# kallenordling/cesm_emulator

Measured on NVIDIA B200. Metric: train samples/s (baseline cfg), higher is better.
Workload: dtype fp16

## Files before the change

cesm_emulator_b200/_lib.py:

```python
from __future__ import annotations

import ctypes
from ctypes import POINTER, Structure, c_char_p, c_float, c_int32, c_int64, c_void_p
from pathlib import Path

_PKG = Path(__file__).resolve().parent
LIB_PATH = _PKG / "libcesm_b200.so"

CESM_MAX_TAPS = 16


class IgemmArgs(Structure):

    _fields_ = [
        ("a0", c_void_p), ("a1", c_void_p),
        ("c0", c_int32), ("c1", c_int32),
        ("n", c_int32), ("h", c_int32), ("w", c_int32),
        ("stride", c_int32),
        ("num_taps", c_int32),
        ("tap_dh", c_int32 * CESM_MAX_TAPS), ("tap_dw", c_int32 * CESM_MAX_TAPS),
        ("wt", c_void_p), ("cout", c_int32),
        ("oh", c_int32), ("ow", c_int32),
        ("out", c_void_p), ("ldo", c_int32),
        ("out_h", c_int32), ("out_w", c_int32),
# ... 62 lines not shown
    lib.cesm_adamw_partials.restype = ctypes.c_int
    lib.cesm_tattn_long_max_frames.restype = ctypes.c_int
    lib.cesm_set_prezeroed_scratch.restype = None
    lib.cesm_set_prezeroed_scratch.argtypes = [ctypes.c_int]
    _declare(lib)
    _lib = lib
    return lib


_P, _I, _L, _F, _U = c_void_p, ctypes.c_int, ctypes.c_longlong, c_float, ctypes.c_uint
_SIGNATURES: dict[str, list] = {
    "cesm_igemm": [POINTER(IgemmArgs), _P],
    "cesm_wgrad": [POINTER(WgradArgs), _P],
    "cesm_pack_weight": [_P, _P, _I, _I, _I, _L, _L, POINTER(c_int32), _P],
    "cesm_pack_weights_batched": [_P, _I, _P],
    "cesm_unpack_wgrads_batched": [_P, _I, _P],
    "cesm_unpack_wgrad": [_P, _P, _I, _I, _I, _L, _L, POINTER(c_int32), _I, _P],
    "cesm_adamw_step": [_P, _P, _P, _P, _L, _P, _P, _F, _F, _F, _F, _P],
    "cesm_adamw_ema_step": [_P, _P, _P, _P, _P, _L, _P, _P, _F, _F, _F, _F, ctypes.c_double, _L, _P],
    "cesm_colsum": [_P, _P, _L, _I, _I, _P],
    "cesm_gn_stats": [_P, _P, _I, _L, _I, _I, _P],
    "cesm_gn_apply_fwd": [_P, _P, _P, _P, _P, _P, _P, _I, _L, _I, _I, _F, _P],
    "cesm_gn_bwd": [_P, _P, _P, _P, _P, _P, _P, _P, _P, _P, _P, _P, _I, _L, _I, _I, _F, _I, _P],
    "cesm_ln_fwd": [_P, _P, _P, _L, _I, _F, _P],
    "cesm_ln_bwd": [_P, _P, _P, _P, _P, _P, _L, _I, _F, _I, _P],
    "cesm_tattn_fwd": [_P, _P, _P, _P, _P, _P, _I, _I, _I, _I, _I, _F, _P],
    "cesm_tattn_bwd": [_P, _P, _P, _P, _P, _P, _P, _P, _P, _I, _I, _I, _I, _I, _F, _P],
    "cesm_tattn_proj_fwd": [_P, _P, _P, _P, _P, _P, _I, _I, _I, _I, _I, _I, _F, _P],
    "cesm_tattn_long_fwd": [_P, _P, _P, _P, _P, _P, _I, _I, _I, _I, _I, _F, _P],
    "cesm_tattn_long_bwd": [_P, _P, _P, _P, _P, _P, _P, _P, _P, _I, _I, _I, _I, _I, _F, _P],
# ... 105 lines not shown
```

cesm_emulator_b200/csrc/api_common.h:

```cpp
#pragma once
#include <cuda.h>
#include <cuda_runtime.h>
#include <stdarg.h>
#include <stdint.h>

#include "../../include/cesm_b200.h"

namespace cesm {

int set_error(int code, const char* fmt, ...);
#define CESM_CHECK_CUDA(expr)                                                                  \
    do {                                                                                       \
        cudaError_t _e = (expr);                                                               \
        if (_e != cudaSuccess)                                                                 \
            return ::cesm::set_error(CESM_ERR_CUDA, "%s failed: %s (%s:%d)", #expr,            \
                                     cudaGetErrorString(_e), __FILE__, __LINE__);              \
    } while (0)
void note_launch();
#define CESM_CHECK_LAUNCH()            \
    do {                               \
        ::cesm::note_launch();         \
        CESM_CHECK_CUDA(cudaGetLastError()); \
    } while (0)
bool scratch_prezeroed();
#define CESM_ZERO_SCRATCH(ptr, bytes, st)                                               \
    do {                                                                                \
        if (!::cesm::scratch_prezeroed()) CESM_CHECK_CUDA(cudaMemsetAsync((ptr), 0, (bytes), (st))); \
    } while (0)
#define CESM_REQUIRE(cond, ...)                                                 \
    do {                                                                        \
        if (!(cond)) return ::cesm::set_error(CESM_ERR_INVALID, __VA_ARGS__);   \
    } while (0)

template <typename... KArgs, typename... Args>
inline cudaError_t launch_pdl(void (*kern)(KArgs...), dim3 grid, dim3 block, size_t smem, cudaStream_t st, Args... args) {
    cudaLaunchConfig_t cfg = {};
    cfg.gridDim = grid;
    cfg.blockDim = block;
    cfg.dynamicSmemBytes = smem;
    cfg.stream = st;
    cudaLaunchAttribute attr[1];
    attr[0].id = cudaLaunchAttributeProgrammaticStreamSerialization;
    attr[0].val.programmaticStreamSerializationAllowed = 1;
    cfg.attrs = attr;
    cfg.numAttrs = 1;
    return cudaLaunchKernelEx(&cfg, kern, static_cast<KArgs>(args)...);
}

template <typename... KArgs, typename... Args>
inline cudaError_t launch_pdl_cluster(void (*kern)(KArgs...), dim3 grid, dim3 block, size_t smem, cudaStream_t st,
                                      int cluster_x, Args... args) {
    cudaLaunchConfig_t cfg = {};
    cfg.gridDim = grid;
    cfg.blockDim = block;
    cfg.dynamicSmemBytes = smem;
    cfg.stream = st;
    cudaLaunchAttribute attr[2];
    attr[0].id = cudaLaunchAttributeProgrammaticStreamSerialization;
    attr[0].val.programmaticStreamSerializationAllowed = 1;
    int n = 1;
    if (cluster_x > 1) {
        attr[n].id = cudaLaunchAttributeClusterDimension;
        attr[n].val.clusterDim.x = (unsigned)cluster_x;
        attr[n].val.clusterDim.y = 1;
        attr[n].val.clusterDim.z = 1;
        ++n;
    }
    cfg.attrs = attr;
    cfg.numAttrs = n;
    return cudaLaunchKernelEx(&cfg, kern, static_cast<KArgs>(args)...);
}

int get_tensor_map_h16(CUtensorMap* out, const void* base, int rank, const uint64_t* dims,
                        const uint64_t* strides_bytes, const uint32_t* box);
// ... 6 lines not shown
```

cesm_emulator_b200/csrc/api_core.cu:

```cuda
#include <atomic>
#include <mutex>
#include <string>
#include <unordered_map>

#include "api_common.h"
#include "igemm.h"

namespace cesm {

static thread_local std::string g_last_error;
static std::atomic<long long> g_launches{0};
void note_launch() { g_launches.fetch_add(1, std::memory_order_relaxed); }
static std::atomic<int> g_prezeroed{0};
bool scratch_prezeroed() { return g_prezeroed.load(std::memory_order_relaxed) != 0; }

int set_error(int code, const char* fmt, ...) {
    char buf[1024];
    va_list ap;
    va_start(ap, fmt);
    vsnprintf(buf, sizeof(buf), fmt, ap);
    va_end(ap);
    g_last_error = buf;
    return code;
}

typedef CUresult (*EncodeTiledFn)(CUtensorMap*, CUtensorMapDataType, cuuint32_t, void*, const cuuint64_t*,
                                  const cuuint64_t*, const cuuint32_t*, const cuuint32_t*, CUtensorMapInterleave,
                                  CUtensorMapSwizzle, CUtensorMapL2promotion, CUtensorMapFloatOOBfill);

// ... 101 lines not shown
        }
    }
    *bw = b_w;
    *bh = b_h;
    *bn = b_n;
}

}

using namespace cesm;

extern "C" const char* cesm_last_error(void) { return g_last_error.c_str(); }
extern "C" const char* cesm_version(void) { return "cesm_b200 0.1 sm_100a"; }
extern "C" void cesm_set_prezeroed_scratch(int on) { g_prezeroed.store(on ? 1 : 0, std::memory_order_relaxed); }
extern "C" long long cesm_launch_count(void) { return g_launches.load(std::memory_order_relaxed); }

static int sm_count() {
    static int n = 0;
    if (n == 0) {
        int dev = 0, v = 0;
        if (cudaGetDevice(&dev) == cudaSuccess &&
            cudaDeviceGetAttribute(&v, cudaDevAttrMultiProcessorCount, dev) == cudaSuccess && v > 0)
            n = v;
        else
            n = 148;
    }
    return n;
}

static bool is_3x3_unit_taps(const cesm_igemm_args* a) {
// ... 73 lines not shown
                     "bad GroupNorm statistics arguments (groups=%d frames=%d)", a->gn_groups, a->gn_frames);
        p.gn_groups = a->gn_groups;
        p.gn_cpg = a->cout / a->gn_groups;
        p.gn_frames = a->gn_frames;
        CESM_REQUIRE(a->gn_groups <= 32, "fused GroupNorm statistics support at most 32 groups (got %d)", a->gn_groups);
        CESM_REQUIRE(p.gn_cpg % 8 == 0 && (p.gn_cpg >= 64 ? p.gn_cpg % 64 == 0 : 64 % p.gn_cpg == 0),
                     "fused GroupNorm statistics need 8 | cout/groups and cout/groups | 64 or 64 | cout/groups (got %d)",
                     p.gn_cpg);
        if (p.bn > 1 && a->gn_frames % p.bn != 0) {
            p.bn = 1;
            p.m_tiles = p.tiles_w * p.tiles_h * a->n;
        }
        CESM_ZERO_SCRATCH(a->gn_sums, sizeof(float) * 2 * (a->n / a->gn_frames) * a->gn_groups, st);
    }

    const int pw = halo ? p.bw + 2 : p.bw;
    if (halo) {
        const int rows_box = pw * (p.bh + 2), rows_need = 2 * pw + 2 + 128;
        const int rows = rows_box > rows_need ? rows_box : rows_need;
        p.a_stage_bytes = (uint32_t)((rows * 128 + 1023) / 1024 * 1024);
        p.a_box_bytes = (uint32_t)rows_box * 128u;
    } else {
        p.a_stage_bytes = 16384;
        p.a_box_bytes = 128u * p.bw * p.bh * p.bn;
    }
    const long long budget = (long long)kIgemm2MaxSmem - 1024  - 1024  - 2 * 16384 ;
    const long long b_total = (long long)a->cout * p.num_kb * 128 / (pair ? 2 : 1);
    const long long b_blk = (long long)block_n * 128 / (pair ? 2 : 1);
    const int a_min = 2;
    if (b_total + a_min * (long long)p.a_stage_bytes <= budget) {
        p.b_resident = 1;
        p.b_stages = 1;
        long long as = (budget - b_total) / p.a_stage_bytes;
        const int a_cap = halo ? 4 : 8;
        p.a_stages = (int)(as > a_cap ? a_cap : as);
    } else {
        p.b_resident = 0;
        p.a_stages = halo ? 2 : 4;
        long long bs = (budget - (long long)p.a_stages * p.a_stage_bytes) / b_blk;
        if (bs > 16) bs = 16;
        if (bs < 2) {
            p.a_stages = 2;
            bs = (budget - (long long)p.a_stages * p.a_stage_bytes) / b_blk;
        }
        CESM_REQUIRE(bs >= 2, "igemm2: no shared-memory plan for cout=%d K=%d", a->cout, p.num_kb * 64);
        p.b_stages = (int)bs;
// ... 72 lines not shown
                                 (uint64_t)a->out_h * a->out_w * a->ldo * 2};
        if (halo)
            p.epi_warp = (pw == 32);
        else
            p.epi_warp = (p.bw % 32 == 0);
        uint32_t obox[4] = {64u, (uint32_t)p.bw, (uint32_t)(halo ? 1 : p.bh), (uint32_t)(halo ? 1 : p.bn)};
        if (p.epi_warp && !halo) {
            obox[1] = 32u;
            obox[2] = 1u;
            obox[3] = 1u;
        }
        int rc = get_tensor_map_h16(&maps.out, base, 4, dims, str, obox);
        if (rc) return rc;
    }
    p.m_major = p.b_resident && p.n_tiles > 1 ? 1 : 0;
    int grid;
    if (pair) {
        const int units = ((p.m_tiles + 1) / 2) * p.n_tiles, clusters = sm_count() / 2;
        grid = 2 * (units < clusters ? units : clusters);
    } else {
        const int total_tiles = p.m_tiles * p.n_tiles;
        grid = total_tiles < sm_count() ? total_tiles : sm_count();
    }
    note_launch();
    CESM_CHECK_CUDA(igemm2_launch(maps, p, block_n, halo, pair, grid, smem, st));
    return CESM_OK;
}

extern "C" int cesm_igemm(const cesm_igemm_args* a, void* stream) {
    CESM_REQUIRE(a != nullptr, "args is NULL");
    CESM_REQUIRE(a->c0 > 0 && a->c0 % 64 == 0 && a->c1 >= 0 && a->c1 % 64 == 0,
                 "channel counts must be multiples of 64 (c0=%d c1=%d)", a->c0, a->c1);
    CESM_REQUIRE(a->cout > 0 && a->cout % 64 == 0, "cout=%d must be a multiple of 64", a->cout);
    CESM_REQUIRE(a->num_taps >= 1 && a->num_taps <= CESM_MAX_TAPS, "num_taps=%d out of range", a->num_taps);
    CESM_REQUIRE(a->stride == 1 || a->stride == 2, "stride=%d unsupported", a->stride);
    CESM_REQUIRE(a->stride == 1 || (a->c1 == 0 && a->h % 2 == 0 && a->w % 2 == 0),
                 "stride 2 needs a single source with even h, w");
    CESM_REQUIRE(a->n > 0 && a->h > 0 && a->w > 0 && a->oh > 0 && a->ow > 0, "empty geometry");
// ... 209 lines not shown
```

cesm_emulator_b200/csrc/elementwise.cu:

```cuda
#include "api_common.h"
#include "common.cuh"

namespace cesm {

struct TapOffsets {
    int32_t off[CESM_MAX_TAPS];
};

__global__ void pack_weight_kernel(const float* __restrict__ src, h16* __restrict__ dst, int O, int T, int I,
                                   long long so, long long si, TapOffsets taps) {
    pdl_trigger();
    pdl_wait();
    const long long idx = (long long)blockIdx.x * blockDim.x + threadIdx.x;
    if (idx >= (long long)O * T * I) return;
    const int i = idx % I;
    const int t = (idx / I) % T;
    const int o = idx / ((long long)I * T);
    dst[idx] = __float2half_rn(src[o * so + i * si + taps.off[t]]);
}
__global__ void unpack_wgrad_kernel(const float* __restrict__ src, float* __restrict__ dst, int O, int T, int I,
                                    long long so, long long si, TapOffsets taps, int accumulate) {
    pdl_trigger();
    pdl_wait();
    const long long idx = (long long)blockIdx.x * blockDim.x + threadIdx.x;
// ... 847 lines not shown

}

using namespace cesm;

static inline int nblk(long long total, int threads) { return (int)((total + threads - 1) / threads); }

extern "C" int cesm_pack_weight(const float* src, void* dst, int O, int T, int I, long long so, long long si,
                                const int32_t* tap_off, void* stream) {
    CESM_REQUIRE(T >= 1 && T <= CESM_MAX_TAPS, "T=%d out of range", T);
    TapOffsets taps{};
    for (int t = 0; t < T; ++t) taps.off[t] = tap_off[t];
    const long long total = (long long)O * T * I;
    launch_pdl(pack_weight_kernel, nblk(total, 256), 256, 0, as_stream(stream), src, (h16*)dst, O, T, I, so, si, taps);
    CESM_CHECK_LAUNCH();
    return CESM_OK;
}

extern "C" int cesm_unpack_wgrad(const float* src, float* dst, int O, int T, int I, long long so, long long si,
                                 const int32_t* tap_off, int accumulate, void* stream) {
    CESM_REQUIRE(T >= 1 && T <= CESM_MAX_TAPS, "T=%d out of range", T);
    TapOffsets taps{};
    for (int t = 0; t < T; ++t) taps.off[t] = tap_off[t];
    const long long total = (long long)O * T * I;
    launch_pdl(unpack_wgrad_kernel, nblk(total, 256), 256, 0, as_stream(stream), src, dst, O, T, I, so, si, taps, accumulate);
    CESM_CHECK_LAUNCH();
    return CESM_OK;
}

extern "C" int cesm_colsum(const void* x, float* out, long long M, int C, int accumulate, void* stream) {
// ... 22 lines not shown
                                  int W, int ks, int kpad, void* stream) {
    CESM_REQUIRE(ks == 7 && kpad == 256, "input patch kernel is specialised for 7x7, 256 columns (ks=%d kpad=%d)", ks, kpad);
    CESM_REQUIRE((f0 == 1 || f0 == F) && (f1 == 1 || f1 == F), "frame counts must be 1 or F");
    dim3 grid(ceil_div(W, 16), ceil_div(H, 16), B * F);
    launch_pdl(input_patches_kernel<7, 256>, grid, 256, 0, as_stream(stream), in0, in1, f0, f1, (h16*)out, F, H, W);
    CESM_CHECK_LAUNCH();
    return CESM_OK;
}

extern "C" int cesm_input_weight_pack(const float* w, const float* bias, void* out, int cout, int ks, int kpad,
                                      void* stream) {
    CESM_REQUIRE(kpad >= 4 * ks * ks + 2, "kpad=%d too small for 2 planes x hi/lo x %dx%d + 2", kpad, ks, ks);
    launch_pdl(input_weight_pack_kernel, nblk((long long)cout * kpad, 256), 256, 0, as_stream(stream), 
        w, bias, (h16*)out, cout, 2 * ks * ks, kpad);
    CESM_CHECK_LAUNCH();
    return CESM_OK;
}

extern "C" int cesm_input_conv_fwd(const float* in0, const float* in1, int f0, int f1, const float* w,
                                   const float* bias, void* out, int B, int F, int H, int W, int ks, int cout,
                                   void* stream) {
    CESM_REQUIRE(ks == 7 && cout == 64, "input conv kernel is specialised for 7x7, 64 channels (ks=%d cout=%d)", ks, cout);
    CESM_REQUIRE((f0 == 1 || f0 == F) && (f1 == 1 || f1 == F), "frame counts must be 1 or F");
    dim3 grid(ceil_div(W, 16), ceil_div(H, 16), B * F);
    launch_pdl(input_conv_fwd_kernel<7, 64>, grid, 256, 0, as_stream(stream), in0, in1, f0, f1, w, bias, (h16*)out, F, H, W);
    CESM_CHECK_LAUNCH();
    return CESM_OK;
}

extern "C" int cesm_input_conv_wgrad(const float* in0, const float* in1, int f0, int f1, const void* dy, float* dw,
// ... 298 lines not shown
```

cesm_emulator_b200/csrc/igemm.h:

```cpp
#pragma once
#include <cuda.h>
#include <cuda_runtime.h>
#include <stdint.h>

namespace cesm {

struct WgradParams {
    int32_t c0, c1;
    int32_t num_taps;
    int32_t tap_map[16];
    int32_t tap_dh[16];
    int32_t tap_dw[16];
    int32_t n, oh, ow;
    int32_t bw, bh, bn;
    uint32_t box_bytes;
    int32_t cout;
    float* dw;
    long long so, si;
    int32_t tap_off[16];
};

struct Wgrad3Maps {
    CUtensorMap x[2];
    CUtensorMap y;
// ... 19 lines not shown
    CUtensorMap b;
    CUtensorMap out;
};

struct Igemm2Params {
    int32_t c0, c1;
    int32_t num_taps, num_kb;
    int32_t tap_map[16];
    int32_t tap_dh[16];
    int32_t tap_dw[16];
    int32_t n, oh, ow;
    int32_t bw, bh, bn;
    int32_t tiles_w, tiles_h, m_tiles, n_tiles;
    int32_t cout;
    int32_t a_stages, b_stages, b_resident;
    uint32_t a_stage_bytes, a_box_bytes;
    int32_t out_h, out_w, o_sh, o_sw, o_h0, o_w0;
    const float* bias;
    const void* residual;
    int32_t ldr;
    float* gn_sums;
    int32_t gn_groups, gn_cpg, gn_frames;
    int32_t epi_warp;
    int32_t m_major;
    const float* ln_colsum;
    float ln_eps;
};

cudaError_t igemm2_launch(const Igemm2Maps& maps, const Igemm2Params& p, int block_n, bool halo, bool pair, int grid,
                          size_t smem, cudaStream_t stream);
// ... 6 lines not shown
```

cesm_emulator_b200/csrc/igemm2.cu:

```cuda

#include "api_common.h"
#include "common.cuh"
#include "igemm.h"

#include <type_traits>

namespace cesm {

static constexpr int kTileM = 128;
static constexpr int kKBlk = 64;
static constexpr int kStageRowBytes = 128;
static constexpr int kOutStageBytes = kTileM * kStageRowBytes;
static constexpr int kIgemm2Threads = 352;

__device__ __forceinline__ void tma_store_4d(const void* map, uint32_t smem_src, int c0, int c1, int c2, int c3) {
    asm volatile("cp.async.bulk.tensor.4d.global.shared::cta.bulk_group [%0, {%2, %3, %4, %5}], [%1];"
                 :
                 : "l"(reinterpret_cast<uint64_t>(map)), "r"(smem_src), "r"(c0), "r"(c1), "r"(c2), "r"(c3)
                 : "memory");
}
__device__ __forceinline__ void tma_store_commit() { asm volatile("cp.async.bulk.commit_group;" ::: "memory"); }
template <int N>
__device__ __forceinline__ void tma_store_wait_read() {
    asm volatile("cp.async.bulk.wait_group.read %0;" ::"n"(N) : "memory");
}
__device__ __forceinline__ void tma_store_wait_all() { asm volatile("cp.async.bulk.wait_group 0;" ::: "memory"); }
__device__ __forceinline__ void epi_bar_sync(int group) {
    asm volatile("bar.sync %0, 128;" ::"r"(group + 1) : "memory");
// ... 23 lines not shown
igemm2_kernel(const __grid_constant__ Igemm2Maps maps, const Igemm2Params p) {
    static_assert(!PAIR || HALO, "CTA pairs are wired for the 3x3 halo mode only");
    static_assert(!LNF || (BLOCK_N == 64 && !HALO && !GN && !PAIR), "the LayerNorm fold is a 64-column plain GEMM epilogue");
    pdl_trigger();
    extern __shared__ uint8_t smem_raw[];
    const uint32_t smem_base = (smem_u32(smem_raw) + 1023u) & ~1023u;
    uint8_t* smem_gen = smem_raw + (smem_base - smem_u32(smem_raw));

    const uint32_t a_base = smem_base;
    const uint32_t b_base = a_base + p.a_stages * p.a_stage_bytes;
    constexpr int kBRows = PAIR ? BLOCK_N / 2 : BLOCK_N;
    const uint32_t b_blk_bytes = kBRows * kStageRowBytes;
    const uint32_t cta_rank = PAIR ? cluster_ctarank() : 0u;
    const int work_id = PAIR ? (int)(blockIdx.x >> 1) : (int)blockIdx.x;
    const int work_stride = PAIR ? (int)(gridDim.x >> 1) : (int)gridDim.x;
    const uint32_t b_bytes = p.b_resident ? (uint32_t)p.n_tiles * p.num_kb * b_blk_bytes : p.b_stages * b_blk_bytes;
    const uint32_t o_base = b_base + b_bytes;
    const uint32_t bar_base = o_base + 2 * kOutStageBytes;
    auto a_full = [&](int s) { return bar_base + 8u * s; };
    auto a_empty = [&](int s) { return bar_base + 8u * (8 + s); };
    auto b_full = [&](int s) { return bar_base + 8u * (16 + s); };
    auto b_empty = [&](int s) { return bar_base + 8u * (32 + s); };
    auto t_full = [&](int s) { return bar_base + 8u * (48 + s); };
    auto t_empty = [&](int s) { return bar_base + 8u * (50 + s); };
    const uint32_t b_all_bar = bar_base + 8u * 52;
    const uint32_t tmem_ptr_addr = bar_base + 8u * 53;
    const uint32_t gn_base = bar_base + 8u * 56;
    volatile uint32_t* tmem_ptr_gen = reinterpret_cast<volatile uint32_t*>(smem_gen + (tmem_ptr_addr - smem_base));

    const int warp = threadIdx.x >> 5;
    const int lane = threadIdx.x & 31;

    const int cblk0 = p.c0 >> 6;
    const int cblk = (p.c0 + p.c1) >> 6;
    const int a_loads = HALO ? cblk : p.num_kb;
    const int taps_per_a = HALO ? 9 : 1;
    const int pw = HALO ? p.bw + 2 : p.bw;
    const int m_units = PAIR ? (p.m_tiles + 1) >> 1 : p.m_tiles;
    const int total_tiles = m_units * p.n_tiles;
    constexpr uint32_t kTmemCols = (2 * BLOCK_N < 32) ? 32 : 2 * BLOCK_N;

    if (threadIdx.x == 0) {
        tma_prefetch_desc(&maps.a[0]);
        tma_prefetch_desc(&maps.b);
        tma_prefetch_desc(&maps.out);
        for (int s = 0; s < p.a_stages; ++s) {
            mbar_init(a_full(s), 1);
            mbar_init(a_empty(s), 1);
        }
        for (int s = 0; s < p.b_stages; ++s) {
            mbar_init(b_full(s), 1);
            mbar_init(b_empty(s), 1);
        }
        for (int s = 0; s < 2; ++s) {
            mbar_init(t_full(s), 1);
            mbar_init(t_empty(s), (BLOCK_N == 64 ? 4 : 8) * (PAIR ? 2 : 1));
        }
        mbar_init(b_all_bar, 1);
        fence_barrier_init();
    }
    if (threadIdx.x < 128) reinterpret_cast<float*>(smem_gen + (gn_base - smem_base))[threadIdx.x] = 0.f;
    if (warp == 2) {
        if (PAIR) tmem_alloc_pair(tmem_ptr_addr, kTmemCols);
        else tmem_alloc(tmem_ptr_addr, kTmemCols);
    }
    tc_fence_before();
    if (PAIR) cluster_sync_all();
    else __syncthreads();
    tc_fence_after();
    const uint32_t tmem_base = *tmem_ptr_gen;

    auto tile_coords = [&](int tile, int& n_tile, int& n0, int& oh0, int& ow0) {
        int t;
// ... 2 lines not shown
            n_tile = tile - t * p.n_tiles;
        } else {
            n_tile = tile / m_units;
            t = tile - n_tile * m_units;
        }
        if (PAIR) t = 2 * t + (int)cta_rank;
        const int tw = t % p.tiles_w;
        t /= p.tiles_w;
        const int th = t % p.tiles_h;
        const int tn = t / p.tiles_h;
        ow0 = tw * p.bw;
        oh0 = th * p.bh;
        n0 = tn * p.bn;
    };

    if (warp == 0 && lane == 0) {
        pdl_wait();
        int stage = 0;
        uint32_t phase = 0;
        for (int tile = work_id; tile < total_tiles; tile += work_stride) {
            int n_tile, n0, oh0, ow0;
            tile_coords(tile, n_tile, n0, oh0, ow0);
            for (int ai = 0; ai < a_loads; ++ai) {
                mbar_wait(a_empty(stage), phase ^ 1u, 11);
                const uint32_t dst = a_base + stage * p.a_stage_bytes;
                if (PAIR) {
                    if (cta_rank == 0) mbar_arrive_expect_tx(a_full(stage), 2 * p.a_box_bytes);
                    int midx = 0, c = ai << 6;
                    if (ai >= cblk0) {
                        midx = 1;
                        c = (ai - cblk0) << 6;
// ... 27 lines not shown
                    stage = 0;
                    phase ^= 1u;
                }
            }
        }
        if (PAIR) {
            for (int k = 0; k < p.a_stages; ++k) {
                mbar_wait(a_empty(stage), phase ^ 1u, 18);
                if (++stage == p.a_stages) {
                    stage = 0;
                    phase ^= 1u;
                }
            }
        }
    } else if (warp == 1 && lane == 0) {
        pdl_wait();
        const int row_off = (int)cta_rank * kBRows;
        if (p.b_resident) {
            const uint32_t total_bytes = (uint32_t)p.n_tiles * p.num_kb * b_blk_bytes;
            if (cta_rank == 0) mbar_arrive_expect_tx(b_all_bar, (PAIR ? 2u : 1u) * total_bytes);
            for (int nt = 0; nt < p.n_tiles; ++nt)
                for (int kb = 0; kb < p.num_kb; ++kb) {
                    const uint32_t dst = b_base + (nt * p.num_kb + kb) * b_blk_bytes;
                    if (PAIR) tma_load_2d_pair(dst, &maps.b, b_all_bar, kb * kKBlk, nt * BLOCK_N + row_off);
                    else tma_load_2d(dst, &maps.b, b_all_bar, kb * kKBlk, nt * BLOCK_N);
                }
        } else {
            int stage = 0;
            uint32_t phase = 0;
            for (int tile = work_id; tile < total_tiles; tile += work_stride) {
                const int n_tile = p.m_major ? tile % p.n_tiles : tile / m_units;
                for (int ai = 0; ai < a_loads; ++ai)
                    for (int ti = 0; ti < taps_per_a; ++ti) {
                        const int kb = HALO ? ti * cblk + ai : ai;
                        mbar_wait(b_empty(stage), phase ^ 1u, 12);
                        if (PAIR) {
                            if (cta_rank == 0) mbar_arrive_expect_tx(b_full(stage), 2 * b_blk_bytes);
                            tma_load_2d_pair(b_base + stage * b_blk_bytes, &maps.b, b_full(stage), kb * kKBlk,
                                             n_tile * BLOCK_N + row_off);
                            if (++stage == p.b_stages) {
                                stage = 0;
                                phase ^= 1u;
                            }
                            continue;
                        }
                        mbar_arrive_expect_tx(b_full(stage), b_blk_bytes);
                        tma_load_2d(b_base + stage * b_blk_bytes, &maps.b, b_full(stage), kb * kKBlk, n_tile * BLOCK_N);
                        if (++stage == p.b_stages) {
                            stage = 0;
                            phase ^= 1u;
                        }
                    }
            }
            if (PAIR) {
                for (int k = 0; k < p.b_stages; ++k) {
                    mbar_wait(b_empty(stage), phase ^ 1u, 19);
                    if (++stage == p.b_stages) {
                        stage = 0;
                        phase ^= 1u;
                    }
                }
            }
        }
    } else if (warp == 2) {
        if (cta_rank == 0 && elect_one()) {
            constexpr uint32_t idesc = make_idesc_f16(PAIR ? 2 * kTileM : kTileM, BLOCK_N, 0, 0);
            const uint64_t desc_hi = make_smem_desc_sw128(0, 0, 1024);
            uint32_t tap_rows8[9];
#pragma unroll
            for (int ti = 0; ti < 9; ++ti)
                tap_rows8[ti] = HALO ? ((1 + p.tap_dh[ti]) * pw + (1 + p.tap_dw[ti])) * 8 : 0;
            const uint32_t b_blk16 = b_blk_bytes >> 4;
            const uint32_t a_stage16 = p.a_stage_bytes >> 4;
            const uint32_t a_base16 = a_base >> 4, b_base16 = b_base >> 4;
            const uint32_t tap_b16 = cblk * b_blk16;
            const uint32_t tile_b16 = p.num_kb * b_blk16;
            const int n_a_stages = p.a_stages, n_b_stages = p.b_stages, n_tiles = p.n_tiles;
            const bool m_major = p.m_major != 0;
            auto mma4 = [&](uint32_t d_tmem, uint32_t a16, uint32_t b16, uint32_t first_accum) {
#pragma unroll
                for (int k = 0; k < kKBlk / 16; ++k) {
                    const uint64_t da = desc_hi | (uint64_t)(a16 + 2 * k), db = desc_hi | (uint64_t)(b16 + 2 * k);
                    if (PAIR) umma_f16_pair(d_tmem, da, db, idesc, k == 0 ? first_accum : 1u);
                    else umma_f16(d_tmem, da, db, idesc, k == 0 ? first_accum : 1u);
                }
            };
            auto commit = [&](uint32_t bar) {
                if (PAIR) umma_commit_pair(bar);
                else umma_commit(bar);
            };
            auto run = [&](auto resident_tag) {
                constexpr bool RES = decltype(resident_tag)::value;
                int a_stage = 0, b_stage = 0, acc = 0;
                uint32_t a_phase = 0, b_phase = 0, acc_phase = 0;
                if (RES) mbar_wait(b_all_bar, 0, 13);
                for (int tile = work_id; tile < total_tiles; tile += work_stride) {
                    const int n_tile = m_major ? tile % n_tiles : tile / m_units;
                    mbar_wait(t_empty(acc), acc_phase ^ 1u, 14);
                    tc_fence_after();
                    const uint32_t d_tmem = tmem_base + acc * BLOCK_N;
                    uint32_t b_kb16 = b_base16 + n_tile * tile_b16;
                    for (int ai = 0; ai < a_loads; ++ai, b_kb16 += b_blk16) {
                        mbar_wait(a_full(a_stage), a_phase, 15);
                        tc_fence_after();
                        const uint32_t sa16 = a_base16 + a_stage * a_stage16;
                        const uint32_t first = ai != 0;
                        if (RES) {
                            if (HALO) {
                                uint32_t b16 = b_kb16;
#pragma unroll
                                for (int ti = 0; ti < 9; ++ti, b16 += tap_b16)
                                    mma4(d_tmem, sa16 + tap_rows8[ti], b16, ti == 0 ? first : 1u);
                            } else {
                                mma4(d_tmem, sa16, b_kb16, first);
                            }
                        } else {
#pragma unroll
                            for (int ti = 0; ti < (HALO ? 9 : 1); ++ti) {
// ... 2 lines not shown
                                mma4(d_tmem, sa16 + tap_rows8[ti], b_base16 + b_stage * b_blk16, ti == 0 ? first : 1u);
                                commit(b_empty(b_stage));
                                if (++b_stage == n_b_stages) {
                                    b_stage = 0;
                                    b_phase ^= 1u;
                                }
                            }
                        }
                        commit(a_empty(a_stage));
                        if (++a_stage == n_a_stages) {
                            a_stage = 0;
                            a_phase ^= 1u;
                        }
                    }
                    commit(t_full(acc));
                    if (++acc == 2) {
                        acc = 0;
                        acc_phase ^= 1u;
                    }
                }
            };
            if (p.b_resident) run(std::true_type{});
            else run(std::false_type{});
        }
        __syncwarp();
    } else if (warp >= 3) {
        const int q = warp & 3;
        const int group = (warp - 3) >> 2;
        const int r = q * 32 + lane;
        const bool grp_issuer = (lane == 0) && (warp == 3 || warp == 7);
        const bool warp_mode = p.epi_warp != 0;
        const uint32_t obuf = o_base + group * kOutStageBytes;
        const uint32_t my_row = obuf + r * kStageRowBytes;
        const uint32_t sw7 = (r & 7);
        float* gn_acc = reinterpret_cast<float*>(smem_gen + (gn_base - smem_base)) + 64 * group;
        int acc = 0;
        uint32_t acc_phase = 0;
        int cur_b = -1;
        auto gn_flush = [&](int b) {
            epi_bar_sync(group);
            if (q == 3 && b >= 0) {
// ... 45 lines not shown
        auto run_flush = [&]() {
            if (run_key < 0) return;
            const int b = run_key / p.n_tiles, nt = run_key - b * p.n_tiles;
            const int col = nt * BLOCK_N + (BLOCK_N == 64 ? 0 : group * 64);
            const int idx = butterfly16(racc);
            if ((lane & 1) == 0) {
                const int g = (col + 8 * (idx & 7)) / p.gn_cpg;
                atomicAdd(p.gn_sums + ((size_t)b * p.gn_groups + g) * 2 + (idx >> 3), racc[0]);
            }
#pragma unroll
            for (int i = 0; i < 16; ++i) racc[i] = 0.f;
        };
        const int rw = r % pw;
        const int rh = (r / pw) % p.bh;
        const int rn = r / (pw * p.bh);
        const int r0 = q * 32;
        const int st_w = HALO ? 0 : r0 % p.bw, st_h = HALO ? q : (r0 / p.bw) % p.bh, st_n = HALO ? 0 : r0 / (p.bw * p.bh);
        const bool st_ok = HALO ? (q < p.bh) : (st_n < p.bn);
        int tile_it = 0;
        for (int tile = work_id; tile < total_tiles; tile += work_stride, ++tile_it) {
            if (BLOCK_N == 64) {
                if ((tile_it & 1) != group) continue;
                acc = group;
                acc_phase = (tile_it >> 1) & 1;
            }
            int n_tile, n0, oh0, ow0;
            tile_coords(tile, n_tile, n0, oh0, ow0);
            if (PAIR && n0 >= p.n) {
                mbar_wait(t_full(acc), acc_phase, 17);
                tc_fence_after();
// ... 13 lines not shown
            if (GN) {
                const int b = n0 / p.gn_frames;
                if (kRunningStats) {
                    const int key = b * p.n_tiles + n_tile;
                    if (key != run_key) {
                        run_flush();
                        run_key = key;
                    }
                } else if (b != cur_b) {
                    if (cur_b >= 0) gn_flush(cur_b);
                    cur_b = b;
                }
            }
            mbar_wait(t_full(acc), acc_phase, 17);
            tc_fence_after();
            const uint32_t taddr = tmem_base + acc * BLOCK_N + (static_cast<uint32_t>(q * 32) << 16);
            const int last_cc = BLOCK_N == 64 ? 0 : group * 64 + (BLOCK_N > 128 ? 128 : 0);
            bool released = false;
#pragma unroll 1
            for (int cc = (BLOCK_N == 64 ? 0 : group * 64); cc < BLOCK_N; cc += 128) {
                uint32_t v[64];
                tmem_ld_32x64(taddr + cc, v);
                if (warp_mode) {
                    if (lane == 0) tma_store_wait_read<0>();
                    __syncwarp();
                } else {
                    if (grp_issuer) tma_store_wait_read<0>();
                    epi_bar_sync(group);
                }
                const int col = n_tile * BLOCK_N + cc;
// ... 180 lines not shown
```

cesm_emulator_b200/csrc/optim.cu:

```cuda
#include "api_common.h"
#include "common.cuh"

namespace cesm {

static constexpr int kRelayoutThreads = 256;
static constexpr int kTile = 32;
static constexpr int kRelayoutSmem = kTile * (kTile * 9 + 1) * (int)sizeof(float);

__device__ __forceinline__ void cp_async4(uint32_t dst, const void* src) {
    asm volatile("cp.async.ca.shared.global [%0], [%1], 4;" ::"r"(dst), "l"(src) : "memory");
}
__device__ __forceinline__ void cp_async_wait_all() { asm volatile("cp.async.wait_all;" ::: "memory"); }

template <int MODE>
__global__ void __launch_bounds__(kRelayoutThreads)
relayout_tiled_kernel(const cesm_pack_desc* __restrict__ descs) {
    pdl_trigger();
    pdl_wait();
    extern __shared__ float tile[];
    __shared__ int s_off[CESM_MAX_TAPS];
    const cesm_pack_desc& d = descs[blockIdx.y];
    const long long so = d.so, si = d.si;
    const int O = d.O, T = d.T, I = d.I;
    const bool inner_is_i = si < so;
// ... 195 lines not shown

static int relayout_launch(const cesm_pack_desc* descs_device, int n, int mode, cudaStream_t st) {
    constexpr int kSmem = kRelayoutSmem;
    static bool cfg = false;
    if (!cfg) {
        CESM_CHECK_CUDA(cudaFuncSetAttribute(relayout_tiled_kernel<0>, cudaFuncAttributeMaxDynamicSharedMemorySize, kSmem));
        CESM_CHECK_CUDA(cudaFuncSetAttribute(relayout_tiled_kernel<1>, cudaFuncAttributeMaxDynamicSharedMemorySize, kSmem));
        cfg = true;
    }
    dim3 grid(32, n);
    if (mode == 0)
        launch_pdl(relayout_tiled_kernel<0>, grid, kRelayoutThreads, kSmem, st, descs_device);
    else
        launch_pdl(relayout_tiled_kernel<1>, grid, kRelayoutThreads, kSmem, st, descs_device);
    CESM_CHECK_LAUNCH();
    return CESM_OK;
}

extern "C" int cesm_pack_weights_batched(const cesm_pack_desc* descs_device, int n, void* stream) {
    if (n <= 0) return CESM_OK;
    return relayout_launch(descs_device, n, 0, as_stream(stream));
}

extern "C" int cesm_unpack_wgrads_batched(const cesm_pack_desc* descs_device, int n, void* stream) {
    if (n <= 0) return CESM_OK;
    return relayout_launch(descs_device, n, 1, as_stream(stream));
}

extern "C" int cesm_adamw_partials(void) { return 148 * 4; }

// ... 35 lines not shown
```

cesm_emulator_b200/kernels.py:

```python
from __future__ import annotations

import ctypes
import numbers
from typing import Optional, Sequence, Tuple

import torch

from . import _lib
from ._lib import IgemmArgs

H16 = torch.float16


def _stream() -> ctypes.c_void_p:
    return ctypes.c_void_p(torch.cuda.current_stream().cuda_stream)


def _ptr(t: Optional[torch.Tensor]) -> Optional[int]:
    return None if t is None else t.data_ptr()


def _req_cuda(*ts: Optional[torch.Tensor]) -> None:
    for t in ts:
        if t is not None and not t.is_cuda:
# ... 406 lines not shown
              h, w, _stream())


INPUT_KPAD = 256


def input_patches(in0, in1, B: int, F: int, H: int, W: int, ks: int) -> torch.Tensor:
    _req_cuda(in0, in1)
    f0, f1 = in0.numel() // (B * H * W), in1.numel() // (B * H * W)
    out = torch.empty((B * F, H, W, INPUT_KPAD), dtype=H16, device=in0.device)
    _lib.call("cesm_input_patches", _ptr(in0), _ptr(in1), f0, f1, _ptr(out), B, F, H, W, ks, INPUT_KPAD, _stream(),
              _meta=_bytes_meta(out))
    return out


def input_weight_pack(w, bias, out: Optional[torch.Tensor] = None) -> torch.Tensor:
    _req_cuda(w, bias)
    cout, ks = w.shape[0], w.shape[-1]
    if out is None:
        out = torch.empty((cout, INPUT_KPAD), dtype=H16, device=w.device)
    _lib.call("cesm_input_weight_pack", _ptr(w), _ptr(bias), _ptr(out), cout, ks, INPUT_KPAD, _stream())
    return out


def input_conv_fwd(in0, in1, w, bias, B: int, F: int, H: int, W: int, ks: int):
    _req_cuda(in0, in1, w, bias)
    cout = w.shape[0]
    f0, f1 = in0.numel() // (B * H * W), in1.numel() // (B * H * W)
    out = torch.empty((B * F, H, W, cout), dtype=H16, device=in0.device)
    _lib.call("cesm_input_conv_fwd", _ptr(in0), _ptr(in1), f0, f1, _ptr(w), _ptr(bias), _ptr(out), B, F, H, W, ks, cout,
# ... 306 lines not shown
```

cesm_emulator_b200/ops.py:

```python
from __future__ import annotations

import weakref
from typing import Optional, Tuple

import torch

from . import _lib
from . import kernels as K

H16 = torch.float16

_PHASE_TAPS = {0: [(0, 1), (-1, 3)], 1: [(1, 0), (0, 2)]}


_OUTER_GRAD = [True]


class _Fn(torch.autograd.Function):
    @classmethod
    def apply(cls, *args, **kwargs):
        _OUTER_GRAD[0] = torch.is_grad_enabled()
        return super().apply(*args, **kwargs)


# ... 95 lines not shown
    return len(live)


_FOLDS: list = []


def _fold_compute(ent, wqkv, wout, gamma) -> None:
    C, hidden = ent[1].shape[0], ent[4]
    wv = wqkv.detach().reshape(3 * hidden, C)[2 * hidden:].float()
    wo = wout.detach().reshape(C, hidden).float()
    w = wo @ wv
    ent[1].copy_(w)
    if gamma is not None:
        ent[6].copy_(w * gamma.detach().reshape(1, C).float())
        ent[7].copy_(ent[6].float().sum(dim=1))


def _fold_f1(meta, wqkv, wout, hidden: int, C: int, gamma=None):
    key = (_key(wqkv), _key(wout), None if gamma is None else _key(gamma))
    ent = meta.__dict__.get("fold_f1")
    if ent is None or ent[1].device != wqkv.device or (gamma is not None and ent[5] is None):
        dev = wqkv.device
        ent = [None, torch.empty((C, C), dtype=H16, device=dev), weakref.ref(wqkv), weakref.ref(wout), hidden,
               None if gamma is None else weakref.ref(gamma),
               None if gamma is None else torch.empty((C, C), dtype=H16, device=dev),
               None if gamma is None else torch.empty((C,), dtype=torch.float32, device=dev)]
        meta.__dict__["fold_f1"] = ent
        _FOLDS.append(ent)
    if ent[0] != key:
        _fold_compute(ent, wqkv, wout, gamma)
# ... 804 lines not shown
```

include/cesm_b200.h:

```cpp
#ifndef CESM_B200_H
#define CESM_B200_H

#include <stddef.h>
#include <stdint.h>

#ifdef __cplusplus
extern "C" {
#endif

typedef enum cesm_status {
    CESM_OK = 0,
    CESM_ERR_INVALID = -1,
    CESM_ERR_CUDA = -2,
    CESM_ERR_INTERNAL = -3
} cesm_status;

const char* cesm_last_error(void);
const char* cesm_version(void);
long long cesm_launch_count(void);


#define CESM_MAX_TAPS 16

typedef struct cesm_igemm_args {
// ... 42 lines not shown
    int32_t dw_tap_off[CESM_MAX_TAPS];
} cesm_wgrad_args;

int cesm_wgrad(const cesm_wgrad_args* args, void* stream);

int cesm_pack_weight(const float* src, void* dst, int O, int T, int I, long long so, long long si,
                     const int32_t* tap_off, void* stream);
typedef struct cesm_pack_desc {
    const float* src;
    void* dst;
    int32_t O, T, I, pad_;
    long long so, si;
    int32_t tap_off[CESM_MAX_TAPS];
} cesm_pack_desc;
int cesm_pack_weights_batched(const cesm_pack_desc* descs_device, int n, void* stream);
int cesm_unpack_wgrads_batched(const cesm_pack_desc* descs_device, int n, void* stream);
int cesm_qkv_bwd(const void* dy, const void* x, const void* wt, void* dx, float* dw, long long dw_so, long long rows,
                 int cin, int cout, void* stream);

void cesm_set_prezeroed_scratch(int on);

#define CESM_OPT_STATE_FLOATS 16
int cesm_adamw_partials(void);
int cesm_adamw_step(float* p, const float* g, float* m, float* v, long long n, float* partials, float* state,
                    float beta1, float beta2, float eps, float max_norm, void* stream);
int cesm_adamw_ema_step(float* p, const float* g, float* m, float* v, float* ema, long long n, float* partials,
                        float* state, float beta1, float beta2, float eps, float max_norm, double ema_decay,
                        long long ema_start, void* stream);
int cesm_unpack_wgrad(const float* src, float* dst, int O, int T, int I, long long so, long long si,
                      const int32_t* tap_off, int accumulate, void* stream);
// ... 112 lines not shown
```

Measured before the change: 190.6.

## Prefetch resident weights before PDL wait and load only needed N tiles

The igemm B-loader warp now issues TMA loads of resident weights before pdl_wait, splitting them across up to 16 per-k-block barriers so MMA can start once the first k-blocks arrive. Each CTA loads only the N tile it needs when the work stride lines up with n_tiles, which shrinks the resident weight footprint. Weight-packing paths record the stream so the next launch there turns off programmatic serialization, keeping the early weight prefetch from reading stale packed weights. The epilogue also prefetches the next tile's residual rows into L2. The cost is extra host mutex bookkeeping per launch and more complex barrier logic.

```diff
diff --git a/cesm_emulator_b200/_lib.py b/cesm_emulator_b200/_lib.py
--- a/cesm_emulator_b200/_lib.py
+++ b/cesm_emulator_b200/_lib.py
@@ -100,6 +100,7 @@
     "cesm_wgrad": [POINTER(WgradArgs), _P],
     "cesm_pack_weight": [_P, _P, _I, _I, _I, _L, _L, POINTER(c_int32), _P],
     "cesm_pack_weights_batched": [_P, _I, _P],
+    "cesm_weights_written": [_P],
     "cesm_unpack_wgrads_batched": [_P, _I, _P],
     "cesm_unpack_wgrad": [_P, _P, _I, _I, _I, _L, _L, POINTER(c_int32), _I, _P],
     "cesm_adamw_step": [_P, _P, _P, _P, _L, _P, _P, _F, _F, _F, _F, _P],
diff --git a/cesm_emulator_b200/csrc/api_common.h b/cesm_emulator_b200/csrc/api_common.h
--- a/cesm_emulator_b200/csrc/api_common.h
+++ b/cesm_emulator_b200/csrc/api_common.h
@@ -32,6 +32,9 @@
         if (!(cond)) return ::cesm::set_error(CESM_ERR_INVALID, __VA_ARGS__);   \
     } while (0)
 
+void note_weight_write(cudaStream_t st);
+bool take_weight_write(cudaStream_t st);
+
 template <typename... KArgs, typename... Args>
 inline cudaError_t launch_pdl(void (*kern)(KArgs...), dim3 grid, dim3 block, size_t smem, cudaStream_t st, Args... args) {
     cudaLaunchConfig_t cfg = {};
@@ -41,7 +44,7 @@
     cfg.stream = st;
     cudaLaunchAttribute attr[1];
     attr[0].id = cudaLaunchAttributeProgrammaticStreamSerialization;
-    attr[0].val.programmaticStreamSerializationAllowed = 1;
+    attr[0].val.programmaticStreamSerializationAllowed = take_weight_write(st) ? 0 : 1;
     cfg.attrs = attr;
     cfg.numAttrs = 1;
     return cudaLaunchKernelEx(&cfg, kern, static_cast<KArgs>(args)...);
@@ -57,7 +60,7 @@
     cfg.stream = st;
     cudaLaunchAttribute attr[2];
     attr[0].id = cudaLaunchAttributeProgrammaticStreamSerialization;
-    attr[0].val.programmaticStreamSerializationAllowed = 1;
+    attr[0].val.programmaticStreamSerializationAllowed = take_weight_write(st) ? 0 : 1;
     int n = 1;
     if (cluster_x > 1) {
         attr[n].id = cudaLaunchAttributeClusterDimension;
diff --git a/cesm_emulator_b200/csrc/api_core.cu b/cesm_emulator_b200/csrc/api_core.cu
--- a/cesm_emulator_b200/csrc/api_core.cu
+++ b/cesm_emulator_b200/csrc/api_core.cu
@@ -2,6 +2,7 @@
 #include <mutex>
 #include <string>
 #include <unordered_map>
+#include <vector>
 
 #include "api_common.h"
 #include "igemm.h"
@@ -13,6 +14,28 @@
 void note_launch() { g_launches.fetch_add(1, std::memory_order_relaxed); }
 static std::atomic<int> g_prezeroed{0};
 bool scratch_prezeroed() { return g_prezeroed.load(std::memory_order_relaxed) != 0; }
+
+static std::mutex g_ww_mutex;
+static std::atomic<int> g_ww_count{0};
+static std::vector<cudaStream_t> g_ww_streams;
+void note_weight_write(cudaStream_t st) {
+    std::lock_guard<std::mutex> lk(g_ww_mutex);
+    for (cudaStream_t s : g_ww_streams)
+        if (s == st) return;
+    g_ww_streams.push_back(st);
+    g_ww_count.store((int)g_ww_streams.size(), std::memory_order_release);
+}
+bool take_weight_write(cudaStream_t st) {
+    if (g_ww_count.load(std::memory_order_acquire) == 0) return false;
+    std::lock_guard<std::mutex> lk(g_ww_mutex);
+    for (size_t i = 0; i < g_ww_streams.size(); ++i)
+        if (g_ww_streams[i] == st) {
+            g_ww_streams.erase(g_ww_streams.begin() + i);
+            g_ww_count.store((int)g_ww_streams.size(), std::memory_order_release);
+            return true;
+        }
+    return false;
+}
 
 int set_error(int code, const char* fmt, ...) {
     char buf[1024];
@@ -144,6 +167,10 @@
 extern "C" const char* cesm_version(void) { return "cesm_b200 0.1 sm_100a"; }
 extern "C" void cesm_set_prezeroed_scratch(int on) { g_prezeroed.store(on ? 1 : 0, std::memory_order_relaxed); }
 extern "C" long long cesm_launch_count(void) { return g_launches.load(std::memory_order_relaxed); }
+extern "C" int cesm_weights_written(void* stream) {
+    note_weight_write(as_stream(stream));
+    return CESM_OK;
+}
 
 static int sm_count() {
     static int n = 0;
@@ -247,6 +274,11 @@
         CESM_ZERO_SCRATCH(a->gn_sums, sizeof(float) * 2 * (a->n / a->gn_frames) * a->gn_groups, st);
     }
 
+    const int units = pair ? ((p.m_tiles + 1) / 2) * p.n_tiles : p.m_tiles * p.n_tiles;
+    const int work_stride = units < (pair ? sm_count() / 2 : sm_count()) ? units : (pair ? sm_count() / 2 : sm_count());
+    const int grid = pair ? 2 * work_stride : work_stride;
+
+    const int b_tiles = (p.n_tiles == 1 || work_stride % p.n_tiles == 0 || units <= work_stride) ? 1 : p.n_tiles;
     const int pw = halo ? p.bw + 2 : p.bw;
     if (halo) {
         const int rows_box = pw * (p.bh + 2), rows_need = 2 * pw + 2 + 128;
@@ -258,11 +290,12 @@
         p.a_box_bytes = 128u * p.bw * p.bh * p.bn;
     }
     const long long budget = (long long)kIgemm2MaxSmem - 1024  - 1024  - 2 * 16384 ;
-    const long long b_total = (long long)a->cout * p.num_kb * 128 / (pair ? 2 : 1);
+    const long long b_total = (long long)b_tiles * block_n * p.num_kb * 128 / (pair ? 2 : 1);
     const long long b_blk = (long long)block_n * 128 / (pair ? 2 : 1);
     const int a_min = 2;
     if (b_total + a_min * (long long)p.a_stage_bytes <= budget) {
         p.b_resident = 1;
+        p.b_tiles = b_tiles;
         p.b_stages = 1;
         long long as = (budget - b_total) / p.a_stage_bytes;
         const int a_cap = halo ? 4 : 8;
@@ -365,14 +398,6 @@
         if (rc) return rc;
     }
     p.m_major = p.b_resident && p.n_tiles > 1 ? 1 : 0;
-    int grid;
-    if (pair) {
-        const int units = ((p.m_tiles + 1) / 2) * p.n_tiles, clusters = sm_count() / 2;
-        grid = 2 * (units < clusters ? units : clusters);
-    } else {
-        const int total_tiles = p.m_tiles * p.n_tiles;
-        grid = total_tiles < sm_count() ? total_tiles : sm_count();
-    }
     note_launch();
     CESM_CHECK_CUDA(igemm2_launch(maps, p, block_n, halo, pair, grid, smem, st));
     return CESM_OK;
diff --git a/cesm_emulator_b200/csrc/elementwise.cu b/cesm_emulator_b200/csrc/elementwise.cu
--- a/cesm_emulator_b200/csrc/elementwise.cu
+++ b/cesm_emulator_b200/csrc/elementwise.cu
@@ -885,6 +885,7 @@
     const long long total = (long long)O * T * I;
     launch_pdl(pack_weight_kernel, nblk(total, 256), 256, 0, as_stream(stream), src, (h16*)dst, O, T, I, so, si, taps);
     CESM_CHECK_LAUNCH();
+    note_weight_write(as_stream(stream));
     return CESM_OK;
 }
 
@@ -937,6 +938,7 @@
     launch_pdl(input_weight_pack_kernel, nblk((long long)cout * kpad, 256), 256, 0, as_stream(stream), 
         w, bias, (h16*)out, cout, 2 * ks * ks, kpad);
     CESM_CHECK_LAUNCH();
+    note_weight_write(as_stream(stream));
     return CESM_OK;
 }
 
diff --git a/cesm_emulator_b200/csrc/igemm.h b/cesm_emulator_b200/csrc/igemm.h
--- a/cesm_emulator_b200/csrc/igemm.h
+++ b/cesm_emulator_b200/csrc/igemm.h
@@ -57,6 +57,7 @@
     int32_t tiles_w, tiles_h, m_tiles, n_tiles;
     int32_t cout;
     int32_t a_stages, b_stages, b_resident;
+    int32_t b_tiles;
     uint32_t a_stage_bytes, a_box_bytes;
     int32_t out_h, out_w, o_sh, o_sw, o_h0, o_w0;
     const float* bias;
diff --git a/cesm_emulator_b200/csrc/igemm2.cu b/cesm_emulator_b200/csrc/igemm2.cu
--- a/cesm_emulator_b200/csrc/igemm2.cu
+++ b/cesm_emulator_b200/csrc/igemm2.cu
@@ -12,6 +12,12 @@
 static constexpr int kStageRowBytes = 128;
 static constexpr int kOutStageBytes = kTileM * kStageRowBytes;
 static constexpr int kIgemm2Threads = 352;
+#ifdef CESM_IGEMM2_PROLOGUE_ONLY
+static constexpr bool kPrologueOnly = true;
+#else
+static constexpr bool kPrologueOnly = false;
+#endif
+static constexpr int kResBars = 16;
 
 __device__ __forceinline__ void tma_store_4d(const void* map, uint32_t smem_src, int c0, int c1, int c2, int c3) {
     asm volatile("cp.async.bulk.tensor.4d.global.shared::cta.bulk_group [%0, {%2, %3, %4, %5}], [%1];"
@@ -65,7 +71,7 @@
     const uint32_t cta_rank = PAIR ? cluster_ctarank() : 0u;
     const int work_id = PAIR ? (int)(blockIdx.x >> 1) : (int)blockIdx.x;
     const int work_stride = PAIR ? (int)(gridDim.x >> 1) : (int)gridDim.x;
-    const uint32_t b_bytes = p.b_resident ? (uint32_t)p.n_tiles * p.num_kb * b_blk_bytes : p.b_stages * b_blk_bytes;
+    const uint32_t b_bytes = p.b_resident ? (uint32_t)p.b_tiles * p.num_kb * b_blk_bytes : p.b_stages * b_blk_bytes;
     const uint32_t o_base = b_base + b_bytes;
     const uint32_t bar_base = o_base + 2 * kOutStageBytes;
     auto a_full = [&](int s) { return bar_base + 8u * s; };
@@ -74,7 +80,6 @@
     auto b_empty = [&](int s) { return bar_base + 8u * (32 + s); };
     auto t_full = [&](int s) { return bar_base + 8u * (48 + s); };
     auto t_empty = [&](int s) { return bar_base + 8u * (50 + s); };
-    const uint32_t b_all_bar = bar_base + 8u * 52;
     const uint32_t tmem_ptr_addr = bar_base + 8u * 53;
     const uint32_t gn_base = bar_base + 8u * 56;
     volatile uint32_t* tmem_ptr_gen = reinterpret_cast<volatile uint32_t*>(smem_gen + (tmem_ptr_addr - smem_base));
@@ -99,7 +104,7 @@
             mbar_init(a_full(s), 1);
             mbar_init(a_empty(s), 1);
         }
-        for (int s = 0; s < p.b_stages; ++s) {
+        for (int s = 0; s < (p.b_resident ? kResBars : p.b_stages); ++s) {
             mbar_init(b_full(s), 1);
             mbar_init(b_empty(s), 1);
         }
@@ -107,7 +112,6 @@
             mbar_init(t_full(s), 1);
             mbar_init(t_empty(s), (BLOCK_N == 64 ? 4 : 8) * (PAIR ? 2 : 1));
         }
-        mbar_init(b_all_bar, 1);
         fence_barrier_init();
     }
     if (threadIdx.x < 128) reinterpret_cast<float*>(smem_gen + (gn_base - smem_base))[threadIdx.x] = 0.f;
@@ -140,7 +144,7 @@
         n0 = tn * p.bn;
     };
 
-    if (warp == 0 && lane == 0) {
+    if (warp == 0 && lane == 0 && !kPrologueOnly) {
         pdl_wait();
         int stage = 0;
         uint32_t phase = 0;
@@ -198,25 +202,37 @@
             }
         }
     } else if (warp == 1 && lane == 0) {
-        pdl_wait();
         const int row_off = (int)cta_rank * kBRows;
         if (p.b_resident) {
-            const uint32_t total_bytes = (uint32_t)p.n_tiles * p.num_kb * b_blk_bytes;
-            if (cta_rank == 0) mbar_arrive_expect_tx(b_all_bar, (PAIR ? 2u : 1u) * total_bytes);
-            for (int nt = 0; nt < p.n_tiles; ++nt)
-                for (int kb = 0; kb < p.num_kb; ++kb) {
-                    const uint32_t dst = b_base + (nt * p.num_kb + kb) * b_blk_bytes;
-                    if (PAIR) tma_load_2d_pair(dst, &maps.b, b_all_bar, kb * kKBlk, nt * BLOCK_N + row_off);
-                    else tma_load_2d(dst, &maps.b, b_all_bar, kb * kKBlk, nt * BLOCK_N);
-                }
-        } else {
-            int stage = 0;
-            uint32_t phase = 0;
-            for (int tile = work_id; tile < total_tiles; tile += work_stride) {
-                const int n_tile = p.m_major ? tile % p.n_tiles : tile / m_units;
-                for (int ai = 0; ai < a_loads; ++ai)
+            const int nt0 = p.b_tiles == 1 ? work_id % p.n_tiles : 0;
+            const uint32_t load_bytes = (uint32_t)(p.b_tiles * taps_per_a) * b_blk_bytes * (PAIR ? 2u : 1u);
+            for (int ai = 0; ai < a_loads; ++ai) {
+                const int g = ai < kResBars - 1 ? ai : kResBars - 1;
+                if (cta_rank == 0 && ai < kResBars)
+                    mbar_arrive_expect_tx(b_full(g), (g < kResBars - 1 ? 1u : (uint32_t)(a_loads - g)) * load_bytes);
+                for (int s = 0; s < p.b_tiles; ++s)
                     for (int ti = 0; ti < taps_per_a; ++ti) {
                         const int kb = HALO ? ti * cblk + ai : ai;
+                        const uint32_t dst = b_base + (s * p.num_kb + kb) * b_blk_bytes;
+                        const int row = (nt0 + s) * BLOCK_N;
+                        if (PAIR) tma_load_2d_pair(dst, &maps.b, b_full(g), kb * kKBlk, row + row_off);
+                        else tma_load_2d(dst, &maps.b, b_full(g), kb * kKBlk, row);
+                    }
+            }
+            pdl_wait();
+        } else {
+            int stage = 0, issued = 0;
+            uint32_t phase = 0;
+            for (int tile = work_id; tile < total_tiles && !(kPrologueOnly && issued >= p.b_stages); tile += work_stride) {
+                const int n_tile = p.m_major ? tile % p.n_tiles : tile / m_units;
+                for (int ai = 0; ai < a_loads && !(kPrologueOnly && issued >= p.b_stages); ++ai)
+                    for (int ti = 0; ti < taps_per_a; ++ti) {
+                        const int kb = HALO ? ti * cblk + ai : ai;
+                        if (issued == p.b_stages) {
+                            if (kPrologueOnly) break;
+                            pdl_wait();
+                        }
+                        ++issued;
                         mbar_wait(b_empty(stage), phase ^ 1u, 12);
                         if (PAIR) {
                             if (cta_rank == 0) mbar_arrive_expect_tx(b_full(stage), 2 * b_blk_bytes);
@@ -236,7 +252,8 @@
                         }
                     }
             }
-            if (PAIR) {
+            if (issued <= p.b_stages) pdl_wait();
+            if (PAIR && !kPrologueOnly) {
                 for (int k = 0; k < p.b_stages; ++k) {
                     mbar_wait(b_empty(stage), phase ^ 1u, 19);
                     if (++stage == p.b_stages) {
@@ -258,7 +275,7 @@
             const uint32_t a_stage16 = p.a_stage_bytes >> 4;
             const uint32_t a_base16 = a_base >> 4, b_base16 = b_base >> 4;
             const uint32_t tap_b16 = cblk * b_blk16;
-            const uint32_t tile_b16 = p.num_kb * b_blk16;
+            const uint32_t tile_b16 = p.b_tiles == 1 ? 0u : p.num_kb * b_blk16;
             const int n_a_stages = p.a_stages, n_b_stages = p.b_stages, n_tiles = p.n_tiles;
             const bool m_major = p.m_major != 0;
             auto mma4 = [&](uint32_t d_tmem, uint32_t a16, uint32_t b16, uint32_t first_accum) {
@@ -277,7 +294,7 @@
                 constexpr bool RES = decltype(resident_tag)::value;
                 int a_stage = 0, b_stage = 0, acc = 0;
                 uint32_t a_phase = 0, b_phase = 0, acc_phase = 0;
-                if (RES) mbar_wait(b_all_bar, 0, 13);
+                bool first_tile = true;
                 for (int tile = work_id; tile < total_tiles; tile += work_stride) {
                     const int n_tile = m_major ? tile % n_tiles : tile / m_units;
                     mbar_wait(t_empty(acc), acc_phase ^ 1u, 14);
@@ -286,6 +303,7 @@
                     uint32_t b_kb16 = b_base16 + n_tile * tile_b16;
                     for (int ai = 0; ai < a_loads; ++ai, b_kb16 += b_blk16) {
                         mbar_wait(a_full(a_stage), a_phase, 15);
+                        if (RES && first_tile) mbar_wait(b_full(ai < kResBars ? ai : kResBars - 1), 0, 13);
                         tc_fence_after();
                         const uint32_t sa16 = a_base16 + a_stage * a_stage16;
                         const uint32_t first = ai != 0;
@@ -318,17 +336,29 @@
                         }
                     }
                     commit(t_full(acc));
+                    first_tile = false;
                     if (++acc == 2) {
                         acc = 0;
                         acc_phase ^= 1u;
                     }
                 }
             };
-            if (p.b_resident) run(std::true_type{});
-            else run(std::false_type{});
+            if (kPrologueOnly) {
+                const int my_tiles = work_id < total_tiles ? (total_tiles - 1 - work_id) / work_stride + 1 : 0;
+                const int loads = my_tiles * a_loads * taps_per_a;
+                if (p.b_resident) {
+                    for (int g = 0; g < a_loads && g < kResBars; ++g) mbar_wait(b_full(g), 0, 13);
+                } else {
+                    for (int st = 0; st < loads && st < n_b_stages; ++st) mbar_wait(b_full(st), 0, 16);
+                }
+            } else if (p.b_resident) {
+                run(std::true_type{});
+            } else {
+                run(std::false_type{});
+            }
         }
         __syncwarp();
-    } else if (warp >= 3) {
+    } else if (warp >= 3 && !kPrologueOnly) {
         const int q = warp & 3;
         const int group = (warp - 3) >> 2;
         const int r = q * 32 + lane;
@@ -404,6 +434,18 @@
         const int rw = r % pw;
         const int rh = (r / pw) % p.bh;
         const int rn = r / (pw * p.bh);
+        auto prefetch_residual = [&](int tile) {
+            int nt, pn0, poh0, pow0;
+            tile_coords(tile, nt, pn0, poh0, pow0);
+            const int pn = pn0 + rn, poh = poh0 + rh, pow_ = pow0 + rw;
+            if (!(rw < p.bw && rn < p.bn && pn < p.n && poh < p.oh && pow_ < p.ow)) return;
+            const long long ppix = (static_cast<long long>(pn) * p.out_h + (poh * p.o_sh + p.o_h0)) * p.out_w +
+                                   (pow_ * p.o_sw + p.o_w0);
+            const h16* row = reinterpret_cast<const h16*>(p.residual) + ppix * p.ldr + nt * BLOCK_N;
+#pragma unroll 1
+            for (int cc = (BLOCK_N == 64 ? 0 : group * 64); cc < BLOCK_N; cc += 128)
+                asm volatile("prefetch.global.L2 [%0];" ::"l"(row + cc) : "memory");
+        };
         const int r0 = q * 32;
         const int st_w = HALO ? 0 : r0 % p.bw, st_h = HALO ? q : (r0 / p.bw) % p.bh, st_n = HALO ? 0 : r0 / (p.bw * p.bh);
         const bool st_ok = HALO ? (q < p.bh) : (st_n < p.bn);
@@ -447,6 +489,10 @@
             }
             mbar_wait(t_full(acc), acc_phase, 17);
             tc_fence_after();
+            if (p.residual != nullptr) {
+                const int next = tile + (BLOCK_N == 64 ? 2 : 1) * work_stride;
+                if (next < total_tiles) prefetch_residual(next);
+            }
             const uint32_t taddr = tmem_base + acc * BLOCK_N + (static_cast<uint32_t>(q * 32) << 16);
             const int last_cc = BLOCK_N == 64 ? 0 : group * 64 + (BLOCK_N > 128 ? 128 : 0);
             bool released = false;
diff --git a/cesm_emulator_b200/csrc/optim.cu b/cesm_emulator_b200/csrc/optim.cu
--- a/cesm_emulator_b200/csrc/optim.cu
+++ b/cesm_emulator_b200/csrc/optim.cu
@@ -233,6 +233,7 @@
     else
         launch_pdl(relayout_tiled_kernel<1>, grid, kRelayoutThreads, kSmem, st, descs_device);
     CESM_CHECK_LAUNCH();
+    if (mode == 0) note_weight_write(st);
     return CESM_OK;
 }
 
diff --git a/cesm_emulator_b200/kernels.py b/cesm_emulator_b200/kernels.py
--- a/cesm_emulator_b200/kernels.py
+++ b/cesm_emulator_b200/kernels.py
@@ -444,6 +444,10 @@
     return out
 
 
+def weights_written() -> None:
+    _lib.check(_lib.load().cesm_weights_written(_stream()), "cesm_weights_written")
+
+
 def input_weight_pack(w, bias, out: Optional[torch.Tensor] = None) -> torch.Tensor:
     _req_cuda(w, bias)
     cout, ks = w.shape[0], w.shape[-1]
diff --git a/cesm_emulator_b200/ops.py b/cesm_emulator_b200/ops.py
--- a/cesm_emulator_b200/ops.py
+++ b/cesm_emulator_b200/ops.py
@@ -133,6 +133,8 @@
     if gamma is not None:
         ent[6].copy_(w * gamma.detach().reshape(1, C).float())
         ent[7].copy_(ent[6].float().sum(dim=1))
+    if ent[1].is_cuda:
+        K.weights_written()
 
 
 def _fold_f1(meta, wqkv, wout, hidden: int, C: int, gamma=None):
diff --git a/include/cesm_b200.h b/include/cesm_b200.h
--- a/include/cesm_b200.h
+++ b/include/cesm_b200.h
@@ -80,6 +80,7 @@
     int32_t tap_off[CESM_MAX_TAPS];
 } cesm_pack_desc;
 int cesm_pack_weights_batched(const cesm_pack_desc* descs_device, int n, void* stream);
+int cesm_weights_written(void* stream);
 int cesm_unpack_wgrads_batched(const cesm_pack_desc* descs_device, int n, void* stream);
 int cesm_qkv_bwd(const void* dy, const void* x, const void* wt, void* dx, float* dw, long long dw_so, long long rows,
                  int cin, int cout, void* stream);
```

Result: no change. 190.5 (median of 6 runs) (-0.0%).
